# arkworks-rs/poly-commit

Measured on NVIDIA H100. Metric: MarlinKZG10/BLS12-381 commit+open polys/s at deg 2^20, higher is better.
Workload: dtype u32-limb Montgomery (Fq 381-bit x12, Fr 255-bit x8)

## Files before the change

poly-commit_b200/csrc/impl.cuh:

```cuda
#pragma once
#include <algorithm>
#include <initializer_list>
#include <memory>
#include <mutex>
#include <new>
#include <type_traits>
#include <vector>

#include "../../include/pcgpu.h"
#include "frops.cuh"
#include "host_ec.hpp"
#include "host_glv.hpp"
#include "ntt.cuh"
#include "ipa.cuh"
#include <chrono>
#include "msm.cuh"
#include "srs.cuh"
#include "wire.cuh"
#include "msm_small.cuh"
#include "peer.cuh"
#include "hash.cuh"
#include "sprs.cuh"
#include "field_ops.cuh"
#include "mlpc.cuh"
// ... 1984 lines not shown
#pragma unroll
      for (int j = 0; j < 8; j++) {
        uint32_t x = hi[(j + 3) & 7];
        lo[j] = mad_lo_cc(x, y, lo[j]);
        hi[j] = madc_hi(x, y, hi[j]);
      }
    }
    uint64_t acc = 0;
#pragma unroll
    for (int j = 0; j < 8; j++) acc ^= ((uint64_t)hi[j] << 32) | lo[j];
    sink[t] = acc;
  }
};

inline int measure_imad_peak_impl(pcgpu_ctx *ctx, double *ops_per_s) {
#ifdef PCGPU_EMUL
  (void)ctx; *ops_per_s = 0; return PCGPU_OK;
#else
  rt::stream_t st = ctx->stream;
  int rc;
  int dev = 0, sms = 0;
  if (cudaGetDevice(&dev) != cudaSuccess || cudaDeviceGetAttribute(&sms, cudaDevAttrMultiProcessorCount, dev) != cudaSuccess)
    return PCGPU_E_CUDA;
  const size_t threads = (size_t)sms * 2048;
  const uint32_t iters = 4096;
  uint64_t *sink;
  Staging io(ctx, 0);
  io.scratch(sink, threads * 8);
  if ((rc = io.upload())) return rc;
  cudaEvent_t e0, e1;
  cudaEventCreate(&e0); cudaEventCreate(&e1);
  if ((rc = rt::launch<256>(ImadPeakBody{sink, 64}, threads, st))) return rc;
  cudaEventRecord(e0, st);
  if ((rc = rt::launch<256>(ImadPeakBody{sink, iters}, threads, st))) return rc;
  cudaEventRecord(e1, st);
  if ((rc = rt::stream_sync(st))) return rc;
  float ms = 0; cudaEventElapsedTime(&ms, e0, e1);
  cudaEventDestroy(e0); cudaEventDestroy(e1);
  *ops_per_s = (double)threads * iters * 8.0 / (ms * 1e-3);
  return PCGPU_OK;
#endif
}

#define PCGPU_INST_PIPE(C, EXT)                                                                                            \
  EXT template int msm_device_planes<C>(pcgpu_ctx *, const MsmPlan &, const uint32_t *, const XYZZ<C> **, uint32_t **);  \
  EXT template int msm_to_host<C>(pcgpu_ctx *, const pcgpu_srs *, size_t, const uint32_t *, size_t, bool, host::HXYZZ<C> *); \
  EXT template int msm_issue<C>(pcgpu_ctx *, const pcgpu_srs *, size_t, const uint32_t *, size_t, bool, MsmPending<C> *);   \
  EXT template int msm_collect<C>(pcgpu_ctx *, MsmPending<C> *, host::HXYZZ<C> *);
#define PCGPU_INST_PAIR1(C, EXT)                                                                                           \
  EXT template int pcgpu::msm_pair_round_oneshot<C>(bool, const uint32_t *, const MsmGeom &, const uint32_t *, const Affine<C> *, uint32_t *, \
                                             const uint32_t *, uint32_t, uint32_t *, const uint32_t *, Affine<C> *, rt::stream_t);   \
  EXT template int pcgpu::msm_pair_oneshot_threads<C>(size_t *);
#define PCGPU_INST_ACC(C, EXT)                                                                                             \
  EXT template int pcgpu::msm_accumulate_launch<C>(const uint32_t *, const MsmGeom &, const uint32_t *, const uint32_t *, const uint32_t *, \
                                            const uint32_t *, XYZZ<C> *, uint32_t *, const Affine<C> *, rt::stream_t);
#define PCGPU_INST_REDUCE(C, EXT)                                                                                          \
  EXT template int pcgpu::msm_reduce_launch<C>(const MsmGeom &, const uint32_t *, const XYZZ<C> *, XYZZ<C> *, XYZZ<C> *, XYZZ<C> *,    \
                                        const uint32_t *, const uint32_t *, rt::stream_t);
#define PCGPU_INST_SMALL(C, EXT)                                                                                           \
  EXT template int msm_small_to_host<C>(pcgpu_ctx *, const MsmPlan &, const MsmSmallProblem<C> *, uint32_t, bool, host::HXYZZ<C> *);
#define PCGPU_INST_SRS(C, EXT)                                                                                             \
  EXT template int srs_register_impl<C>(pcgpu_ctx *, const void *, const uint8_t *, size_t, uint32_t, pcgpu_srs *);        \
  EXT template int msm_impl<C>(pcgpu_ctx *, const pcgpu_srs *, size_t, const void *, size_t, uint32_t, void *, uint8_t *, void *); \
  EXT template int g1_sum_impl<C>(pcgpu_ctx *, const void *, size_t, void *, uint8_t *);                                   \
  EXT template int fixed_base_impl<C>(pcgpu_ctx *, const void *, const void *, size_t, uint32_t, void *);                  \
  EXT template int kzg_commit_impl<C>(pcgpu_ctx *, const pcgpu_srs *, const void *, size_t, const pcgpu_srs *, const void *, \
                                      size_t, uint32_t, void *, uint8_t *);                                                \
  EXT template int kzg_open_impl<C>(pcgpu_ctx *, const pcgpu_srs *, const void *, size_t, const void *, const pcgpu_srs *, \
                                    const void *, size_t, uint32_t, void *, uint8_t *, void *); \
  EXT template int msm_batch_impl<C>(pcgpu_ctx *, const pcgpu_srs *, const void *, size_t, size_t, uint32_t, void *, uint8_t *); \
  EXT template int kzg_commit_open_impl<C>(pcgpu_ctx *, pcgpu_ctx *, const pcgpu_srs *, const void *, size_t, const void *, uint32_t, void *, uint8_t *, void *, uint8_t *); \
  EXT template int msm_peer_impl<C>(pcgpu_ctx *, const pcgpu_srs *, size_t, const void *, size_t, uint32_t, void *const *, uint32_t, uint32_t, uint64_t, void *, uint8_t *); \
  EXT template int hyrax_commit_impl<C>(pcgpu_ctx *, const pcgpu_srs *, uint32_t, const void *, const void *, uint32_t, void *, uint8_t *, pcgpu_hyrax *); \
  EXT template int hyrax_open_impl<C>(pcgpu_ctx *, const pcgpu_srs *, const pcgpu_hyrax *const *, size_t, uint32_t, const void *, const void *, \
                                      uint32_t, void *, uint8_t *, void *, void *); \
  EXT template int hyrax_check_impl<C>(pcgpu_ctx *, const pcgpu_srs *, uint32_t, size_t, const void *, const uint8_t *, const void *, const void *, \
                                       const uint8_t *, const void *, const void *, uint32_t, uint8_t *);
#define PCGPU_INST_FR(C, EXT)                                                                                              \
  EXT template int fr_from_mont_impl<C>(pcgpu_ctx *, const void *, void *, size_t, uint32_t);                              \
  EXT template int fr_axpy_impl<C>(pcgpu_ctx *, void *, const void *, const void *, size_t, uint32_t);                     \
  EXT template int fr_div_impl<C>(pcgpu_ctx *, const void *, size_t, const void *, void *, void *, uint32_t);              \
  EXT template int fr_ip_impl<C>(pcgpu_ctx *, const void *, const void *, size_t, void *, uint32_t);                       \
  EXT template int fr_row_mul_impl<C>(pcgpu_ctx *, const void *, const void *, size_t, size_t, void *, uint32_t);          \
  EXT template int fr_mul_impl<C>(pcgpu_ctx *, const void *, const void *, void *, size_t, uint32_t); \
  EXT template int selftest_field_impl<C>(pcgpu_ctx *, uint64_t, size_t, uint64_t *); \
  EXT template int diag_field_op_impl<C>(pcgpu_ctx *, int, int, const void *, const void *, void *, size_t); \
  EXT template int ntt_impl<C>(pcgpu_ctx *, const void *, size_t, uint32_t, uint32_t, void *); \
  EXT template int ntt_pass_impl<C>(pcgpu_ctx *, uint32_t, uint32_t, int, size_t, size_t, const void *, size_t, void *); \
  EXT template int ntt_batch_impl<C>(pcgpu_ctx *, const void *, size_t, size_t, uint32_t, uint32_t, void *); \
  EXT template int ntt_pass1_peer_impl<C>(pcgpu_ctx *, uint32_t, uint32_t, size_t, size_t, const void *, size_t, void *const *, uint32_t); \
  EXT template int lincode_hash_columns_impl<C>(pcgpu_ctx *, const void *, size_t, size_t, int, uint32_t, uint8_t *); \
  EXT template int lincode_commit_impl<C>(pcgpu_ctx *, const void *, size_t, size_t, uint32_t, int, uint32_t, void *, uint8_t *, uint8_t *, uint8_t *); \
  EXT template int brakedown_register_impl<C>(pcgpu_ctx *, uint64_t, uint64_t, uint64_t, const uint64_t *, const uint64_t *, \
                                              const uint64_t *const *, const uint64_t *const *, const void *const *, pcgpu_brakedown *); \
  EXT template int brakedown_commit_impl<C>(pcgpu_ctx *, const pcgpu_brakedown *, const void *, size_t, size_t, int, uint32_t, void *, \
                                            uint8_t *, uint8_t *, uint8_t *); \
  EXT template int fr_sprs_row_mul_impl<C>(pcgpu_ctx *, size_t, size_t, const uint64_t *, const uint64_t *, const void *, const void *, \
                                           size_t, uint32_t, void *);
#define PCGPU_INST_IPA(C, EXT)                                                                                             \
  EXT template int ipa_begin_impl<C>(pcgpu_ctx *, const void *, size_t, const void *, size_t, const void *, uint32_t, pcgpu_ipa *); \
  EXT template int ipa_round_lr_impl<C>(pcgpu_ctx *, pcgpu_ctx *, pcgpu_ipa *, const void *, void *, uint8_t *, void *, uint8_t *); \
  EXT template int ipa_round_fold_impl<C>(pcgpu_ctx *, pcgpu_ipa *, const void *, const void *); \
  EXT template int ipa_finish_impl<C>(pcgpu_ctx *, pcgpu_ipa *, void *, void *); \
  EXT template int ipa_check_final_key_impl<C>(pcgpu_ctx *, const pcgpu_srs *, const void *, uint32_t, void *, uint8_t *); \
  EXT template int g1_serialize_impl<C>(pcgpu_ctx *, const void *, const uint8_t *, size_t, uint32_t, uint8_t *); \
  EXT template int g1_deserialize_impl<C>(pcgpu_ctx *, const uint8_t *, size_t, uint32_t, void *, uint8_t *, size_t *, int *); \
  EXT template int g1_sample_generators_impl<C>(pcgpu_ctx *, const uint8_t *, size_t, uint64_t, size_t, uint32_t, void *);
#define PCGPU_INST_G2(C, EXT)                                                                                              \
  EXT template int srs_register_impl<C>(pcgpu_ctx *, const void *, const uint8_t *, size_t, uint32_t, pcgpu_srs *);        \
  EXT template int msm_impl<C>(pcgpu_ctx *, const pcgpu_srs *, size_t, const void *, size_t, uint32_t, void *, uint8_t *, void *); \
  EXT template int fixed_base_impl<C>(pcgpu_ctx *, const void *, const void *, size_t, uint32_t, void *);                  \
// ... 16 lines not shown
```

poly-commit_b200/csrc/msm.cuh:

```cuda
#pragma once
#include "ec.cuh"
#include "rt.cuh"

namespace pcgpu {

struct alignas(16) u32x4 { uint32_t x, y, z, w; };

struct MsmGeom {
  uint32_t n;
  uint32_t c;
  uint32_t W;
  uint32_t S;
  uint32_t G;
  uint32_t NB;
  uint32_t TB;
  uint32_t L;
  uint32_t seg_len;
  uint32_t nseg;
  uint32_t scalar_bits;
  uint32_t scalars_mont;
  uint64_t table_stride;
  uint64_t base_off;
  uint32_t affine_rounds;
  uint32_t h_split;
// ... 135 lines not shown
    size_t lo = t * SCAN_CHUNK, hi = lo + SCAN_CHUNK < n ? lo + SCAN_CHUNK : n;
    uint32_t run = partial[t];
    for (size_t i = lo; i < hi; i++) { uint32_t v = in[i]; out[i] = run; run += v; }
    if (t + 1 == m) out[n] = partial[m];
  }
};

enum { SCAN_BLOCK = 1024, SCAN_PER = 8, SCAN_BLOCK_MAX = 1 << 17 };
struct ScanBlockBody {
  const uint32_t *in; size_t n; uint32_t *out;
  PCGPU_KERNEL_DEV void operator()(size_t, uint32_t *smem) const {
    uint32_t *a = smem, *b = smem + SCAN_BLOCK, *carry = smem + 2 * SCAN_BLOCK;
    PCGPU_BLOCK_FOR(t, 1) { carry[0] = 0; }
    PCGPU_BLOCK_SYNC();
    const size_t tile = (size_t)SCAN_BLOCK * SCAN_PER;
    for (size_t base = 0; base < n; base += tile) {
      PCGPU_BLOCK_FOR(t, SCAN_BLOCK) {
        const size_t lo = base + (size_t)t * SCAN_PER;
        uint32_t sum = 0;
        for (uint32_t k = 0; k < SCAN_PER; k++) if (lo + k < n) sum += in[lo + k];
        a[t] = sum;
      }
      PCGPU_BLOCK_SYNC();
      uint32_t *x = a, *y = b;
      for (uint32_t d = 1; d < SCAN_BLOCK; d <<= 1) {
        PCGPU_BLOCK_FOR(t, SCAN_BLOCK) { y[t] = x[t] + (t >= d ? x[t - d] : 0u); }
        PCGPU_BLOCK_SYNC();
        uint32_t *tmp = x; x = y; y = tmp;
      }
      PCGPU_BLOCK_FOR(t, SCAN_BLOCK) {
        const size_t lo = base + (size_t)t * SCAN_PER;
        uint32_t run = carry[0] + (t ? x[t - 1] : 0u);
        for (uint32_t k = 0; k < SCAN_PER; k++) if (lo + k < n) { uint32_t v = in[lo + k]; out[lo + k] = run; run += v; }
      }
      PCGPU_BLOCK_SYNC();
      PCGPU_BLOCK_FOR(t, 1) { carry[0] += x[SCAN_BLOCK - 1]; }
      PCGPU_BLOCK_SYNC();
    }
    PCGPU_BLOCK_FOR(t, 1) { out[n] = carry[0]; }
  }
};

inline size_t scan_scratch_words(size_t n) { return (n + SCAN_CHUNK - 1) / SCAN_CHUNK + 2; }
inline int exclusive_scan_u32(const uint32_t *in, size_t n, uint32_t *out, uint32_t *scratch, rt::stream_t st) {
  size_t m = (n + SCAN_CHUNK - 1) / SCAN_CHUNK;
  if (m == 0) { return rt::dev_memset(out, 0, sizeof(uint32_t), st); }
  if (n <= SCAN_BLOCK_MAX) return rt::launch_blocks<SCAN_BLOCK>(ScanBlockBody{in, n, out}, 1, (2 * SCAN_BLOCK + 4) * sizeof(uint32_t), st);
  int rc;
  if ((rc = rt::launch<128>(ScanChunkSumBody{in, n, scratch}, m, st))) return rc;
  if ((rc = rt::launch<32>(ScanPartialsBody{scratch, m}, 1, st))) return rc;
  return rt::launch<128>(ScanApplyBody{in, n, scratch, out, m}, m, st);
}

struct TaskCountBody {
  const uint32_t *offsets; uint32_t L; uint32_t *ntasks; uint32_t heavy_min; uint32_t *heavy_count; uint32_t *heavy_list;
  PCGPU_KERNEL_DEV void operator()(size_t b) const {
    uint32_t cnt = offsets[b + 1] - offsets[b];
    uint32_t nt = (cnt + L - 1) / L;
    ntasks[b] = nt;
    if (nt > heavy_min) heavy_list[rt::atomic_add(heavy_count, 1u)] = (uint32_t)b;
  }
};
struct TaskFillBody {
  const uint32_t *task_off; uint32_t *task_bucket;
  PCGPU_KERNEL_DEV void operator()(size_t b) const {
    uint32_t lo = task_off[b], hi = task_off[b + 1];
    for (uint32_t t = lo; t < hi; t++) task_bucket[t] = (uint32_t)b;
  }
};

template <class C>
PCGPU_DEV Affine<C> load_affine(const Affine<C> *p) {
  constexpr int N = coord_words<typename C::F>();
  const u32x4 *q = reinterpret_cast<const u32x4 *>(p);
  Affine<C> a;
  uint32_t tmp[2 * N];
#pragma unroll
  for (int j = 0; j < 2 * N / 4; j++) { u32x4 v = q[j]; tmp[4 * j] = v.x; tmp[4 * j + 1] = v.y; tmp[4 * j + 2] = v.z; tmp[4 * j + 3] = v.w; }
#pragma unroll
  for (int j = 0; j < N; j++) {
    if constexpr (C::EXT == 1) { a.x.l[j] = tmp[j]; a.y.l[j] = tmp[N + j]; }
    else { coord_word(a.x, j) = tmp[j]; coord_word(a.y, j) = tmp[N + j]; }
  }
  return a;
}

template <class C>
PCGPU_DEV const uint32_t *table_record(const uint32_t *tables, size_t idx, const MsmGeom &g) { return tables + idx * g.pt_words; }
template <class C>
PCGPU_DEV Affine<C> load_table_point(const uint32_t *tables, size_t idx, const MsmGeom &g) {
  constexpr int N = coord_words<typename C::F>();
  const uint32_t *rec = tables + idx * g.pt_words;
  const u32x4 *qx = reinterpret_cast<const u32x4 *>(rec), *qy = reinterpret_cast<const u32x4 *>(rec + g.y_words);
  Affine<C> a;
#pragma unroll
  for (int j = 0; j < N / 4; j++) {
    u32x4 v = qx[j]; coord_word(a.x, 4 * j) = v.x; coord_word(a.x, 4 * j + 1) = v.y; coord_word(a.x, 4 * j + 2) = v.z; coord_word(a.x, 4 * j + 3) = v.w;
    u32x4 w = qy[j]; coord_word(a.y, 4 * j) = w.x; coord_word(a.y, 4 * j + 1) = w.y; coord_word(a.y, 4 * j + 2) = w.z; coord_word(a.y, 4 * j + 3) = w.w;
  }
  return a;
}
template <class C>
PCGPU_DEV void store_table_point(uint32_t *tables, size_t idx, uint32_t pt_words, uint32_t y_words, const Affine<C> &a) {
  constexpr int N = coord_words<typename C::F>();
  uint32_t *rec = tables + idx * pt_words;
  u32x4 *qx = reinterpret_cast<u32x4 *>(rec), *qy = reinterpret_cast<u32x4 *>(rec + y_words);
#pragma unroll
  for (int j = 0; j < N / 4; j++) {
    u32x4 v; v.x = coord_word(a.x, 4 * j); v.y = coord_word(a.x, 4 * j + 1); v.z = coord_word(a.x, 4 * j + 2); v.w = coord_word(a.x, 4 * j + 3); qx[j] = v;
    u32x4 w; w.x = coord_word(a.y, 4 * j); w.y = coord_word(a.y, 4 * j + 1); w.z = coord_word(a.y, 4 * j + 2); w.w = coord_word(a.y, 4 * j + 3); qy[j] = w;
  }
}
template <class C> constexpr uint32_t aligned_pt_words() { return C::Fq::N == 12 ? 32u : 2u * C::Fq::N; }
template <class C> constexpr uint32_t aligned_y_words() { return C::Fq::N == 12 ? 16u : (uint32_t)C::Fq::N; }

template <class C>
PCGPU_DEV void store_xyzz(XYZZ<C> *dst, const XYZZ<C> &p) {
  constexpr int N = coord_words<typename C::F>();
  u32x4 *q = reinterpret_cast<u32x4 *>(dst);
  const uint32_t *src = reinterpret_cast<const uint32_t *>(&p);
#pragma unroll
  for (int j = 0; j < 4 * N / 4; j++) { u32x4 v; v.x = src[4 * j]; v.y = src[4 * j + 1]; v.z = src[4 * j + 2]; v.w = src[4 * j + 3]; q[j] = v; }
}

template <class C>
PCGPU_DEV XYZZ<C> load_xyzz(const XYZZ<C> *src) {
  constexpr int N = coord_words<typename C::F>();
  const u32x4 *q = reinterpret_cast<const u32x4 *>(src);
  XYZZ<C> p;
  uint32_t *dst = reinterpret_cast<uint32_t *>(&p);
#pragma unroll
  for (int j = 0; j < 4 * N / 4; j++) { u32x4 v = q[j]; dst[4 * j] = v.x; dst[4 * j + 1] = v.y; dst[4 * j + 2] = v.z; dst[4 * j + 3] = v.w; }
  return p;
}

template <class C>
struct MsmAccumulateBody {
  const uint32_t *tables; MsmGeom g;
  const uint32_t *offsets;
  const uint32_t *task_off;
  const uint32_t *task_bucket;
  const uint32_t *entries;
  XYZZ<C> *partial;
  uint32_t *queue;
  const Affine<C> *pts;
  PCGPU_KERNEL_DEV void operator()(size_t) const {
    const uint32_t total = task_off[g.TB];
    for (;;) {
      uint32_t t = rt::next_task(queue);
      if (t - (t & 31u) >= total) break;
      if (t >= total) continue;
      uint32_t b = task_bucket[t];
      uint32_t t0 = task_off[b], T = task_off[b + 1] - t0, j = t - t0;
      uint32_t base = offsets[b], cnt = offsets[b + 1] - base;
      uint32_t lo = base + (uint32_t)(((uint64_t)cnt * j) / T);
      uint32_t hi = base + (uint32_t)(((uint64_t)cnt * (j + 1)) / T);
      XYZZ<C> acc = XYZZ<C>::inf();
      if (pts) {
        for (uint32_t e = lo; e < hi; e++) { Affine<C> a = load_affine<C>(pts + e); xyzz_madd<C>(acc, a, false); }
      } else {
        for (uint32_t e = lo; e < hi; e++) {
          uint32_t v = entries[e];
          uint32_t grp = (v & ~ENTRY_SIGN) >> ENTRY_GROUP_SHIFT;
          size_t idx = (size_t)grp * g.table_stride + g.base_off + (v & ENTRY_IDX_MASK);
          Affine<C> a = load_table_point<C>(tables, idx, g);
          xyzz_madd<C>(acc, a, (v & ENTRY_SIGN) != 0);
        }
      }
      store_xyzz<C>(partial + t, acc);
    }
  }
};

enum { HEAVY_BUCKET_TASKS = 8, HEAVY_BLOCK = 128, HEAVY_GRID = 64, REDUCE_BLOCK = 128 };

template <class C>
#ifdef __CUDACC__
__device__ __noinline__
#else
inline
#endif
void xyzz_add_ool(XYZZ<C> &acc, const XYZZ<C> &p) { xyzz_add<C>(acc, p); }

template <class C>
struct MsmHeavyBucketBody {
  const uint32_t *task_off; const XYZZ<C> *partial; XYZZ<C> *buckets; const uint32_t *heavy_count; const uint32_t *heavy_list;
  PCGPU_KERNEL_DEV void operator()(size_t blk, uint32_t *smem) const {
    XYZZ<C> *sh = reinterpret_cast<XYZZ<C> *>(smem);
    const uint32_t nheavy = *heavy_count;
    for (uint32_t hb = (uint32_t)blk; hb < nheavy; hb += HEAVY_GRID) {
      const uint32_t b = heavy_list[hb], t0 = task_off[b], t1 = task_off[b + 1];
      PCGPU_BLOCK_FOR(i, HEAVY_BLOCK) {
        XYZZ<C> acc = XYZZ<C>::inf();
#pragma unroll 1
        for (uint32_t q = t0 + i; q < t1; q += HEAVY_BLOCK) { XYZZ<C> p = load_xyzz<C>(partial + q); xyzz_add_ool<C>(acc, p); }
        sh[i] = acc;
      }
      PCGPU_BLOCK_SYNC();
#pragma unroll 1
      for (uint32_t half = HEAVY_BLOCK / 2; half >= 1; half >>= 1) {
        PCGPU_BLOCK_FOR(i, half) { XYZZ<C> x = sh[i], y = sh[i + half]; xyzz_add_ool<C>(x, y); sh[i] = x; }
        PCGPU_BLOCK_SYNC();
      }
      PCGPU_BLOCK_FOR(i, 1) { store_xyzz<C>(buckets + b, sh[0]); }
      PCGPU_BLOCK_SYNC();
    }
  }
};

template <class C>
PCGPU_KERNEL_DEV void block_tree_sum(XYZZ<C> *sh) {
#pragma unroll 1
  for (uint32_t half = REDUCE_BLOCK / 2; half >= 1; half >>= 1) {
    PCGPU_BLOCK_FOR(i, half) { XYZZ<C> x = sh[i], y = sh[i + half]; xyzz_add_ool<C>(x, y); sh[i] = x; }
    PCGPU_BLOCK_SYNC();
  }
}

template <class C>
struct MsmRowReduceBody {
  const uint32_t *task_off; const XYZZ<C> *partial; XYZZ<C> *buckets; XYZZ<C> *Rv;
  uint32_t NB, rows, cols;
  PCGPU_KERNEL_DEV void operator()(size_t blk, uint32_t *smem) const {
    XYZZ<C> *sh = reinterpret_cast<XYZZ<C> *>(smem);
    const uint32_t s = (uint32_t)(blk / rows), hi = (uint32_t)(blk % rows);
    PCGPU_BLOCK_FOR(t, REDUCE_BLOCK) {
      XYZZ<C> acc = XYZZ<C>::inf();
#pragma unroll 1
      for (uint32_t lo = t; lo < cols; lo += REDUCE_BLOCK) {
        const size_t b = (size_t)s * NB + (size_t)hi * cols + lo;
        const uint32_t t0 = task_off[b], t1 = task_off[b + 1];
        XYZZ<C> bs;
        if (t1 - t0 > HEAVY_BUCKET_TASKS) bs = load_xyzz<C>(buckets + b);
        else {
          bs = XYZZ<C>::inf();
#pragma unroll 1
          for (uint32_t q = t0; q < t1; q++) { XYZZ<C> p = load_xyzz<C>(partial + q); xyzz_add_ool<C>(bs, p); }
          store_xyzz<C>(buckets + b, bs);
        }
        xyzz_add_ool<C>(acc, bs);
      }
      sh[t] = acc;
    }
    PCGPU_BLOCK_SYNC();
    block_tree_sum<C>(sh);
    PCGPU_BLOCK_FOR(i, 1) { store_xyzz<C>(Rv + blk, sh[0]); }
  }
};
template <class C>
struct MsmColReduceBody {
  const XYZZ<C> *buckets; XYZZ<C> *Cv;
  uint32_t NB, rows, cols;
  PCGPU_KERNEL_DEV void operator()(size_t blk, uint32_t *smem) const {
    XYZZ<C> *sh = reinterpret_cast<XYZZ<C> *>(smem);
    const uint32_t s = (uint32_t)(blk / cols), lo = (uint32_t)(blk % cols);
    PCGPU_BLOCK_FOR(t, REDUCE_BLOCK) {
      XYZZ<C> acc = XYZZ<C>::inf();
#pragma unroll 1
      for (uint32_t hi = t; hi < rows; hi += REDUCE_BLOCK) {
        XYZZ<C> p = load_xyzz<C>(buckets + (size_t)s * NB + (size_t)hi * cols + lo);
        xyzz_add_ool<C>(acc, p);
      }
      sh[t] = acc;
    }
    PCGPU_BLOCK_SYNC();
    block_tree_sum<C>(sh);
    PCGPU_BLOCK_FOR(i, 1) { store_xyzz<C>(Cv + blk, sh[0]); }
  }
};
template <class C>
struct MsmPlaneReduceBody {
  const XYZZ<C> *Rv, *Cv; XYZZ<C> *plane_out;
  uint32_t rows, cols, bits_c, bits_r;
  PCGPU_KERNEL_DEV void operator()(size_t blk, uint32_t *smem) const {
    XYZZ<C> *sh = reinterpret_cast<XYZZ<C> *>(smem);
    const uint32_t per = bits_c + bits_r;
    const uint32_t s = (uint32_t)(blk / per), j = (uint32_t)(blk % per);
    const bool col = j < bits_c;
    const XYZZ<C> *vals = col ? Cv + (size_t)s * cols : Rv + (size_t)s * rows;
    const uint32_t cnt = col ? cols : rows, wofs = col ? 1u : 0u, bit = col ? j : j - bits_c;
    PCGPU_BLOCK_FOR(t, REDUCE_BLOCK) {
      XYZZ<C> acc = XYZZ<C>::inf();
#pragma unroll 1
      for (uint32_t k = t; k < cnt; k += REDUCE_BLOCK)
        if (((k + wofs) >> bit) & 1) { XYZZ<C> p = load_xyzz<C>(vals + k); xyzz_add_ool<C>(acc, p); }
      sh[t] = acc;
    }
// ... 22 lines not shown
  MsmGeom g{};
  g.n = (uint32_t)n; g.c = c;
  g.W = (scalar_bits + c - 1) / c;
  g.G = groups < 1 ? 1 : groups;
  g.S = (g.W + g.G - 1) / g.G;
  g.NB = 1u << (c - 1);
  g.TB = g.S * g.NB;
  g.L = L;
  g.seg_len = 16;
  g.nseg = (g.NB + g.seg_len - 1) / g.seg_len;
  g.scalar_bits = scalar_bits; g.scalars_mont = mont ? 1 : 0;
  g.table_stride = table_stride; g.base_off = base_off;
  g.h_split = (c - 1) / 2;
  return g;
}

struct MsmPlan {
  uint32_t path;
  uint64_t n;
  uint32_t split;
  MsmGeom g;
  const uint32_t *tables;
  size_t wave;
  uint32_t T;
};

inline size_t msm_plane_scratch_elems(const MsmGeom &g) {
  size_t cols = (size_t)1 << g.h_split, rows = g.NB >> g.h_split;
  return (size_t)g.S * (rows + cols);
}

enum {
  MSM_ERR_RANGE = 0,
  MSM_ERR_QUEUE = 8,
  MSM_ERR_HEAVY = 12,
  MSM_ERR_WORDS = 16,
};

#ifndef PCGPU_PAIR_MIN_BLOCKS
#define PCGPU_PAIR_MIN_BLOCKS 4
#endif
enum { PAIR_MIN_BLOCKS = PCGPU_PAIR_MIN_BLOCKS };

template <class C>
int msm_pair_round_oneshot(bool round0, const uint32_t *tables, const MsmGeom &g, const uint32_t *entries, const Affine<C> *in,
                           uint32_t *src, const uint32_t *off_out, uint32_t T, uint32_t *prefix, const uint32_t *pow2, Affine<C> *out,
                           rt::stream_t st) {
  if (round0) return rt::launch_occ<128, PAIR_MIN_BLOCKS>(MsmAffinePairBody<C, true>{tables, g, entries, nullptr, src, off_out, T, prefix, pow2, out}, T, st);
  return rt::launch_occ<128, PAIR_MIN_BLOCKS>(MsmAffinePairBody<C, false>{tables, g, entries, in, src, off_out, T, prefix, pow2, out}, T, st);
}
template <class C> int msm_pair_oneshot_threads(size_t *out) { return rt::resident_threads_occ<128, PAIR_MIN_BLOCKS, MsmAffinePairBody<C, true>>(out); }

template <class C>
int msm_accumulate_launch(const uint32_t *tables, const MsmGeom &g, const uint32_t *offsets, const uint32_t *task_off,
                          const uint32_t *task_bucket, const uint32_t *entries, XYZZ<C> *partial, uint32_t *queue, const Affine<C> *pts,
                          rt::stream_t st) {
  return rt::launch_persistent<128>(MsmAccumulateBody<C>{tables, g, offsets, task_off, task_bucket, entries, partial, queue, pts}, st);
}

template <class C>
int msm_reduce_launch(const MsmGeom &g, const uint32_t *task_off, const XYZZ<C> *partial, XYZZ<C> *buckets, XYZZ<C> *planes,
                      XYZZ<C> *plane_out, const uint32_t *heavy_count, const uint32_t *heavy_list, rt::stream_t st) {
  const uint32_t h = g.h_split, cols = 1u << h, rows = g.NB >> h, bits_c = h + 1, bits_r = g.c - 1 - h;
  const size_t smem = REDUCE_BLOCK * sizeof(XYZZ<C>);
  XYZZ<C> *Rv = planes, *Cv = planes + (size_t)g.S * rows;
  int rc;
  if ((rc = rt::launch_blocks<HEAVY_BLOCK>(MsmHeavyBucketBody<C>{task_off, partial, buckets, heavy_count, heavy_list}, HEAVY_GRID,
                                           HEAVY_BLOCK * sizeof(XYZZ<C>), st))) return rc;
  if ((rc = rt::launch_blocks<REDUCE_BLOCK>(MsmRowReduceBody<C>{task_off, partial, buckets, Rv, g.NB, rows, cols}, (size_t)g.S * rows, smem, st))) return rc;
  if ((rc = rt::launch_blocks<REDUCE_BLOCK>(MsmColReduceBody<C>{buckets, Cv, g.NB, rows, cols}, (size_t)g.S * cols, smem, st))) return rc;
  return rt::launch_blocks<REDUCE_BLOCK>(MsmPlaneReduceBody<C>{Rv, Cv, plane_out, rows, cols, bits_c, bits_r}, (size_t)g.S * (bits_c + bits_r), smem, st);
}

template <class C, class Prof>
inline int msm_run(const MsmPlan &plan, const uint32_t *d_scalars, rt::Arena &arena, const XYZZ<C> **d_planes,
                   uint32_t **d_err_out, rt::stream_t st, Prof &prof, const uint32_t *pow2) {
  using QF = Fp<typename C::Fq>;
  const MsmGeom &g = plan.g;
  const size_t max_entries = (size_t)g.n * g.W, max_tasks = max_entries / g.L + g.TB + 1;
  const size_t bound0 = max_entries / 2 + g.TB + 1, bound1 = bound0 / 2 + g.TB + 1;
  const bool pair_rounds = C::EXT == 1 && g.affine_rounds;
  uint32_t *counts, *offsets, *cursor, *ntasks, *task_off, *task_bucket, *entries, *scratch, *err;
  XYZZ<C> *partial, *buckets, *planes, *plane_out;
  uint32_t *offA = nullptr, *offB = nullptr, *cnt = nullptr, *src = nullptr;
  QF *prefix = nullptr; Affine<C> *ptsA = nullptr, *ptsB = nullptr;
  int rc = arena.carve([&](auto &&buf) {
    buf(counts, g.TB + 2); buf(offsets, g.TB + 2); buf(cursor, g.TB + 2); buf(ntasks, g.TB + 2); buf(task_off, g.TB + 2);
    buf(task_bucket, max_tasks); buf(entries, max_entries + 1); buf(scratch, scan_scratch_words(g.TB + 1)); buf(err, MSM_ERR_WORDS);
    buf(partial, max_tasks); buf(buckets, g.TB); buf(planes, msm_plane_scratch_elems(g));
    buf(plane_out, (size_t)g.S * 2 * g.c);
    if (pair_rounds) {
      buf(offA, g.TB + 2); buf(offB, g.TB + 2); buf(cnt, g.TB + 2); buf(src, bound0);
      buf(prefix, bound0 + (1u << 20));
      buf(ptsA, bound0); buf(ptsB, bound1);
    }
  });
  if (rc) return rc;
  *d_err_out = err; *d_planes = plane_out;

  prof.begin(0, st);
  if ((rc = rt::dev_memset(counts, 0, (g.TB + 2) * sizeof(uint32_t), st))) return rc;
  if ((rc = rt::dev_memset(err, 0, MSM_ERR_WORDS * sizeof(uint32_t), st))) return rc;
  if ((rc = rt::launch<256>(MsmCountBody<C>{d_scalars, g, counts, err + MSM_ERR_RANGE}, g.n, st))) return rc;
  prof.end(0, st);

  prof.begin(1, st);
  if ((rc = exclusive_scan_u32(counts, g.TB, offsets, scratch, st))) return rc;
  if ((rc = rt::copy_d2d(cursor, offsets, (g.TB + 1) * sizeof(uint32_t), st))) return rc;
  prof.end(1, st);

  prof.begin(2, st);
  if ((rc = rt::launch<256>(MsmScatterBody<C>{d_scalars, g, cursor, entries}, g.n, st))) return rc;
  prof.end(2, st);

  const Affine<C> *pts = nullptr;
  if constexpr (C::EXT == 1) if (pair_rounds) {
    prof.begin(11, st);
    const uint32_t *off_in = offsets;
    size_t bound = max_entries;
    for (uint32_t r = 0; r < g.affine_rounds; r++) {
      uint32_t *off_out = (r & 1) ? offB : offA;
      Affine<C> *out = (r & 1) ? ptsB : ptsA;
      const Affine<C> *in = (r & 1) ? ptsA : ptsB;
      bound = bound / 2 + g.TB + 1;
      if ((rc = rt::launch<256>(PairCountBody{off_in, cnt}, g.TB, st))) return rc;
      if ((rc = exclusive_scan_u32(cnt, g.TB, off_out, scratch, st))) return rc;
      if ((rc = rt::launch<256>(PairPlanBody{off_in, off_out, g.TB, src}, bound, st))) return rc;
      if (r == 0) prof.begin(12, st);
      rc = msm_pair_round_oneshot<C>(r == 0, plan.tables, g, entries, in, src, off_out, plan.T, (uint32_t *)prefix, pow2, out, st);
      if (rc) return rc;
      if (r == 0) prof.end(12, st);
      off_in = off_out;
      pts = out;
    }
    prof.end(11, st);
    offsets = const_cast<uint32_t *>(off_in);
  }

  prof.begin(3, st);
  if ((rc = rt::dev_memset(err + MSM_ERR_HEAVY, 0, 4, st))) return rc;
  if ((rc = rt::launch<256>(TaskCountBody{offsets, g.L, ntasks, HEAVY_BUCKET_TASKS, err + MSM_ERR_HEAVY, cursor}, g.TB, st))) return rc;
  if ((rc = exclusive_scan_u32(ntasks, g.TB, task_off, scratch, st))) return rc;
  if ((rc = rt::launch<256>(TaskFillBody{task_off, task_bucket}, g.TB, st))) return rc;
  prof.end(3, st);

  prof.begin(4, st);
  if ((rc = msm_accumulate_launch<C>(plan.tables, g, offsets, task_off, task_bucket, entries, partial, err + MSM_ERR_QUEUE, pts, st))) return rc;
  prof.end(4, st);

  prof.begin(5, st);
  if ((rc = msm_reduce_launch<C>(g, task_off, partial, buckets, planes, plane_out, err + MSM_ERR_HEAVY, cursor, st))) return rc;
  prof.end(5, st);
  return rt::OK;
}

}
```

poly-commit_b200/csrc/rt.cuh:

```cuda
#pragma once
#include <stddef.h>
#include <stdint.h>
#include <stdlib.h>
#include <string.h>
#include <atomic>
#include <type_traits>

#ifndef PCGPU_EMUL
#include <cuda_runtime.h>
#endif

namespace pcgpu {
namespace rt {

enum : int {
  OK = 0,
  E_CUDA = -1,
  E_OOM = -2,
  E_BADARG = -3,
  E_LEN = -4,
  E_RANGE = -5,
  E_DEGREE = -6,
  E_HIDING = -7,
};

inline std::atomic<uint64_t> &launch_counter() { static std::atomic<uint64_t> c{0}; return c; }

#ifdef PCGPU_EMUL
typedef void *stream_t;
inline int dev_malloc(void **p, size_t bytes) { *p = ::malloc(bytes ? bytes : 1); return *p ? OK : E_OOM; }
inline void dev_free(void *p) { ::free(p); }
inline int dev_memset(void *p, int v, size_t bytes, stream_t) { memset(p, v, bytes); return OK; }
inline int copy_h2d(void *d, const void *h, size_t bytes, stream_t) { memcpy(d, h, bytes); return OK; }
inline int copy_d2h(void *h, const void *d, size_t bytes, stream_t) { memcpy(h, d, bytes); return OK; }
inline int copy_d2d(void *d, const void *s, size_t bytes, stream_t) { memmove(d, s, bytes); return OK; }
inline int stream_sync(stream_t) { return OK; }
inline int last_error() { return OK; }
typedef int event_t;
inline int event_create(event_t *e) { *e = 0; return OK; }
inline void event_destroy(event_t) {}
inline int event_record(event_t, stream_t) { return OK; }
inline int stream_wait_event(stream_t, event_t) { return OK; }
inline int host_alloc_pinned(void **p, size_t bytes) { *p = ::malloc(bytes ? bytes : 1); return *p ? OK : E_OOM; }
inline void host_free_pinned(void *p) { ::free(p); }

template <int BLOCK, class Body>
inline int launch(const Body &body, size_t n, stream_t) {
  for (size_t i = 0; i < n; i++) body(i);
  return OK;
}
template <class T> inline T atomic_add(T *p, T v) { T o = *p; *p = o + v; return o; }
template <class T> inline T atomic_or(T *p, T v) { T o = *p; *p = o | v; return o; }
#define PCGPU_KERNEL_DEV inline
inline uint32_t next_task(uint32_t *counter) { return atomic_add(counter, 1u); }
template <int BLOCK, class Body>
inline int launch_persistent(const Body &body, stream_t) { body(0); return OK; }
template <int BLOCK, int MINB, class Body> inline int launch_occ(const Body &body, size_t n, stream_t s) { return launch<BLOCK>(body, n, s); }
template <int BLOCK, int MINB, class Body> inline int resident_threads_occ(size_t *out) { *out = 48; return OK; }
#define PCGPU_BLOCK_FOR(i, n) for (uint32_t i = 0; i < (uint32_t)(n); i++)
#define PCGPU_BLOCK_SYNC() do { } while (0)
#define PCGPU_WARP_ANY(x) (x)
template <int BLOCK, class Body>
inline int launch_blocks(const Body &body, size_t nblocks, size_t smem_bytes, stream_t) {
  uint32_t *smem = (uint32_t *)::malloc(smem_bytes ? smem_bytes : 16);
  if (!smem) return E_OOM;
  for (size_t b = 0; b < nblocks; b++) body(b, smem);
  ::free(smem);
  return OK;
}

template <int BLOCK, int MINB, class Body>
inline int launch_blocks_occ(const Body &body, size_t nblocks, size_t smem_bytes, stream_t s) { return launch_blocks<BLOCK>(body, nblocks, smem_bytes, s); }

#else
typedef cudaStream_t stream_t;

inline int map_cuda(cudaError_t e) {
  if (e == cudaSuccess) return OK;
  if (e == cudaErrorMemoryAllocation) return E_OOM;
  return E_CUDA;
}
inline int dev_malloc(void **p, size_t bytes) { return map_cuda(cudaMalloc(p, bytes ? bytes : 1)); }
inline void dev_free(void *p) { if (p) cudaFree(p); }
inline int dev_memset(void *p, int v, size_t bytes, stream_t s) { return map_cuda(cudaMemsetAsync(p, v, bytes, s)); }
inline int copy_h2d(void *d, const void *h, size_t bytes, stream_t s) { return map_cuda(cudaMemcpyAsync(d, h, bytes, cudaMemcpyHostToDevice, s)); }
inline int copy_d2h(void *h, const void *d, size_t bytes, stream_t s) { return map_cuda(cudaMemcpyAsync(h, d, bytes, cudaMemcpyDeviceToHost, s)); }
inline int copy_d2d(void *d, const void *s_, size_t bytes, stream_t s) { return map_cuda(cudaMemcpyAsync(d, s_, bytes, cudaMemcpyDeviceToDevice, s)); }
inline int stream_sync(stream_t s) { return map_cuda(cudaStreamSynchronize(s)); }
inline int last_error() { return map_cuda(cudaGetLastError()); }
typedef cudaEvent_t event_t;
inline int event_create(event_t *e) { return map_cuda(cudaEventCreateWithFlags(e, cudaEventDisableTiming)); }
inline void event_destroy(event_t e) { cudaEventDestroy(e); }
inline int event_record(event_t e, stream_t s) { return map_cuda(cudaEventRecord(e, s)); }
inline int stream_wait_event(stream_t s, event_t e) { return map_cuda(cudaStreamWaitEvent(s, e, 0)); }
inline int host_alloc_pinned(void **p, size_t bytes) { return map_cuda(cudaMallocHost(p, bytes ? bytes : 1)); }
inline void host_free_pinned(void *p) { if (p) cudaFreeHost(p); }

template <class Body, int BLOCK>
__global__ void __launch_bounds__(BLOCK) run_kernel(const Body body, size_t n) {
  size_t tid = (size_t)blockIdx.x * BLOCK + threadIdx.x;
  if (tid < n) body(tid);
}

template <int BLOCK, class Body>
inline int launch(const Body &body, size_t n, stream_t s) {
  if (n == 0) return OK;
  size_t grid = (n + BLOCK - 1) / BLOCK;
  run_kernel<Body, BLOCK><<<(unsigned)grid, BLOCK, 0, s>>>(body, n);
  launch_counter().fetch_add(1, std::memory_order_relaxed);
// ... 22 lines not shown
    if (e == cudaSuccess) e = cudaOccupancyMaxActiveBlocksPerMultiprocessor(&per_sm, run_kernel_occ<Body, BLOCK, MINB>, BLOCK, 0);
    if (e != cudaSuccess) return map_cuda(e);
    cached = (size_t)sms * (per_sm > 0 ? per_sm : 1) * BLOCK;
  }
  *out = cached;
  return OK;
}
#define PCGPU_BLOCK_FOR(i, n) for (uint32_t i = threadIdx.x; i < (uint32_t)(n); i += blockDim.x)
#define PCGPU_BLOCK_SYNC() __syncthreads()
#define PCGPU_WARP_ANY(x) __any_sync(0xffffffffu, (x))
template <class Body, int BLOCK>
__global__ void __launch_bounds__(BLOCK) run_block_kernel(const Body body) {
  extern __shared__ uint4 pcgpu_smem[];
  body((size_t)blockIdx.x, reinterpret_cast<uint32_t *>(pcgpu_smem));
}
template <int BLOCK, class Body>
inline int launch_blocks(const Body &body, size_t nblocks, size_t smem_bytes, stream_t s) {
  if (nblocks == 0) return OK;
  if (smem_bytes > 48 * 1024) {
    cudaError_t e = cudaFuncSetAttribute(run_block_kernel<Body, BLOCK>, cudaFuncAttributeMaxDynamicSharedMemorySize, (int)smem_bytes);
    if (e != cudaSuccess) return map_cuda(e);
  }
  run_block_kernel<Body, BLOCK><<<(unsigned)nblocks, BLOCK, smem_bytes, s>>>(body);
  launch_counter().fetch_add(1, std::memory_order_relaxed);
  return last_error();
}
template <class Body, int BLOCK, int MINB>
__global__ void __launch_bounds__(BLOCK, MINB) run_block_kernel_occ(const Body body) {
  extern __shared__ uint4 pcgpu_smem[];
  body((size_t)blockIdx.x, reinterpret_cast<uint32_t *>(pcgpu_smem));
}
template <int BLOCK, int MINB, class Body>
inline int launch_blocks_occ(const Body &body, size_t nblocks, size_t smem_bytes, stream_t s) {
  if (nblocks == 0) return OK;
  if (smem_bytes > 48 * 1024) {
    cudaError_t e = cudaFuncSetAttribute(run_block_kernel_occ<Body, BLOCK, MINB>, cudaFuncAttributeMaxDynamicSharedMemorySize, (int)smem_bytes);
    if (e != cudaSuccess) return map_cuda(e);
  }
  run_block_kernel_occ<Body, BLOCK, MINB><<<(unsigned)nblocks, BLOCK, smem_bytes, s>>>(body);
  launch_counter().fetch_add(1, std::memory_order_relaxed);
  return last_error();
}
__device__ __forceinline__ uint32_t next_task(uint32_t *counter) {
  uint32_t lane = threadIdx.x & 31, base = 0;
  if (lane == 0) base = atomicAdd(counter, 32u);
  base = __shfl_sync(0xffffffffu, base, 0);
  return base + lane;
}
template <class Body, int BLOCK>
__global__ void __launch_bounds__(BLOCK) run_persistent_kernel(const Body body) {
  body((size_t)blockIdx.x * BLOCK + threadIdx.x);
}
template <int BLOCK, class Body>
inline int launch_persistent(const Body &body, stream_t s) {
  static int grid = 0;
  if (grid == 0) {
    int dev = 0, sms = 0, per_sm = 0;
    cudaError_t e = cudaGetDevice(&dev);
    if (e == cudaSuccess) e = cudaDeviceGetAttribute(&sms, cudaDevAttrMultiProcessorCount, dev);
    if (e == cudaSuccess) e = cudaOccupancyMaxActiveBlocksPerMultiprocessor(&per_sm, run_persistent_kernel<Body, BLOCK>, BLOCK, 0);
    if (e != cudaSuccess) return map_cuda(e);
    grid = sms * (per_sm > 0 ? per_sm : 1);
  }
  run_persistent_kernel<Body, BLOCK><<<grid, BLOCK, 0, s>>>(body);
  launch_counter().fetch_add(1, std::memory_order_relaxed);
  return last_error();
}
template <class T> __device__ __forceinline__ T atomic_add(T *p, T v) { return atomicAdd(p, v); }
template <class T> __device__ __forceinline__ T atomic_or(T *p, T v) { return atomicOr(p, v); }
#define PCGPU_KERNEL_DEV __device__ __forceinline__
#endif

struct Arena {
  char *base = nullptr;
  size_t cap = 0;
  int reserve(size_t bytes) {
    if (bytes <= cap) return OK;
    if (base) dev_free(base);
    base = nullptr; cap = 0;
    int rc = dev_malloc((void **)&base, bytes);
    if (rc) return rc;
    cap = bytes;
    return OK;
  }
  template <class List> int carve(const List &list) {
    size_t used = 0;
    list([&](auto *&p, size_t count) { used += padded(sizeof *p, count); });
    int rc = reserve(used);
    if (rc) return rc;
    used = 0;
    list([&](auto *&p, size_t count) {
      p = reinterpret_cast<std::remove_reference_t<decltype(p)>>(base + used);
      used += padded(sizeof *p, count);
    });
    return OK;
  }
  static size_t padded(size_t elem, size_t count) { size_t b = elem * count; return ((b ? b : 1) + 255) & ~(size_t)255; }
  void release() { if (base) dev_free(base); base = nullptr; cap = 0; }
};

}
}
```

Before: 74.52.

## Split MSM bucket accumulation into equal flat chunks across persistent lanes

```diff
diff --git a/poly-commit_b200/csrc/impl.cuh b/poly-commit_b200/csrc/impl.cuh
--- a/poly-commit_b200/csrc/impl.cuh
+++ b/poly-commit_b200/csrc/impl.cuh
@@ -2060,11 +2060,12 @@
                                              const uint32_t *, uint32_t, uint32_t *, const uint32_t *, Affine<C> *, rt::stream_t);   \
   EXT template int pcgpu::msm_pair_oneshot_threads<C>(size_t *);
 #define PCGPU_INST_ACC(C, EXT)                                                                                             \
-  EXT template int pcgpu::msm_accumulate_launch<C>(const uint32_t *, const MsmGeom &, const uint32_t *, const uint32_t *, const uint32_t *, \
-                                            const uint32_t *, XYZZ<C> *, uint32_t *, const Affine<C> *, rt::stream_t);
+  EXT template int pcgpu::msm_accumulate_launch<C>(const uint32_t *, const MsmGeom &, const uint32_t *, const uint32_t *, XYZZ<C> *, \
+                                            uint32_t *, const Affine<C> *, uint32_t, rt::stream_t);                        \
+  EXT template int pcgpu::msm_tail_chunks<C>(uint32_t *);
 #define PCGPU_INST_REDUCE(C, EXT)                                                                                          \
-  EXT template int pcgpu::msm_reduce_launch<C>(const MsmGeom &, const uint32_t *, const XYZZ<C> *, XYZZ<C> *, XYZZ<C> *, XYZZ<C> *,    \
-                                        const uint32_t *, const uint32_t *, rt::stream_t);
+  EXT template int pcgpu::msm_reduce_launch<C>(const MsmGeom &, const uint32_t *, uint32_t, const XYZZ<C> *, XYZZ<C> *, XYZZ<C> *, \
+                                        XYZZ<C> *, const uint32_t *, const uint32_t *, rt::stream_t);
 #define PCGPU_INST_SMALL(C, EXT)                                                                                           \
   EXT template int msm_small_to_host<C>(pcgpu_ctx *, const MsmPlan &, const MsmSmallProblem<C> *, uint32_t, bool, host::HXYZZ<C> *);
 #define PCGPU_INST_SRS(C, EXT)                                                                                             \
diff --git a/poly-commit_b200/csrc/msm.cuh b/poly-commit_b200/csrc/msm.cuh
--- a/poly-commit_b200/csrc/msm.cuh
+++ b/poly-commit_b200/csrc/msm.cuh
@@ -211,20 +211,23 @@
   return rt::launch<128>(ScanApplyBody{in, n, scratch, out, m}, m, st);
 }
 
-struct TaskCountBody {
-  const uint32_t *offsets; uint32_t L; uint32_t *ntasks; uint32_t heavy_min; uint32_t *heavy_count; uint32_t *heavy_list;
+enum { TAIL_CHUNKS_PER_LANE = 1, HEAVY_BUCKET_TASKS = 8 };
+
+PCGPU_DEV uint32_t tail_chunk_len(uint32_t M, uint32_t chunks, uint32_t L) {
+  const uint32_t s = M / chunks + (M % chunks != 0), lo = L / 2;
+  return s > lo ? s : lo;
+}
+PCGPU_DEV void tail_partials(const uint32_t *offsets, uint32_t b, uint32_t s, uint32_t *t0, uint32_t *t1) {
+  const uint32_t lo = offsets[b], hi = offsets[b + 1];
+  *t0 = lo / s + b;
+  *t1 = lo < hi ? (hi - 1) / s + b + 1 : *t0;
+}
+PCGPU_DEV bool tail_heavy(uint32_t cnt, uint32_t L) { return (cnt + L - 1) / L > HEAVY_BUCKET_TASKS; }
+
+struct HeavyListBody {
+  const uint32_t *offsets; uint32_t L; uint32_t *heavy_count; uint32_t *heavy_list;
   PCGPU_KERNEL_DEV void operator()(size_t b) const {
-    uint32_t cnt = offsets[b + 1] - offsets[b];
-    uint32_t nt = (cnt + L - 1) / L;
-    ntasks[b] = nt;
-    if (nt > heavy_min) heavy_list[rt::atomic_add(heavy_count, 1u)] = (uint32_t)b;
-  }
-};
-struct TaskFillBody {
-  const uint32_t *task_off; uint32_t *task_bucket;
-  PCGPU_KERNEL_DEV void operator()(size_t b) const {
-    uint32_t lo = task_off[b], hi = task_off[b + 1];
-    for (uint32_t t = lo; t < hi; t++) task_bucket[t] = (uint32_t)b;
+    if (tail_heavy(offsets[b + 1] - offsets[b], L)) heavy_list[rt::atomic_add(heavy_count, 1u)] = (uint32_t)b;
   }
 };
 
@@ -297,41 +300,45 @@
 struct MsmAccumulateBody {
   const uint32_t *tables; MsmGeom g;
   const uint32_t *offsets;
-  const uint32_t *task_off;
-  const uint32_t *task_bucket;
   const uint32_t *entries;
   XYZZ<C> *partial;
   uint32_t *queue;
   const Affine<C> *pts;
+  uint32_t chunks;
   PCGPU_KERNEL_DEV void operator()(size_t) const {
-    const uint32_t total = task_off[g.TB];
+    const uint32_t M = offsets[g.TB], s = tail_chunk_len(M, chunks, g.L), total = M / s + (M % s != 0);
     for (;;) {
-      uint32_t t = rt::next_task(queue);
+      const uint32_t t = rt::next_task(queue);
       if (t - (t & 31u) >= total) break;
       if (t >= total) continue;
-      uint32_t b = task_bucket[t];
-      uint32_t t0 = task_off[b], T = task_off[b + 1] - t0, j = t - t0;
-      uint32_t base = offsets[b], cnt = offsets[b + 1] - base;
-      uint32_t lo = base + (uint32_t)(((uint64_t)cnt * j) / T);
-      uint32_t hi = base + (uint32_t)(((uint64_t)cnt * (j + 1)) / T);
+      const uint32_t lo = t * s, hi = M - lo > s ? lo + s : M;
+      uint32_t b = 0, bh = g.TB;
+      while (bh - b > 1) { const uint32_t mid = (b + bh) >> 1; if (offsets[mid] <= lo) b = mid; else bh = mid; }
+      uint32_t next = offsets[b + 1];
       XYZZ<C> acc = XYZZ<C>::inf();
-      if (pts) {
-        for (uint32_t e = lo; e < hi; e++) { Affine<C> a = load_affine<C>(pts + e); xyzz_madd<C>(acc, a, false); }
-      } else {
-        for (uint32_t e = lo; e < hi; e++) {
-          uint32_t v = entries[e];
-          uint32_t grp = (v & ~ENTRY_SIGN) >> ENTRY_GROUP_SHIFT;
-          size_t idx = (size_t)grp * g.table_stride + g.base_off + (v & ENTRY_IDX_MASK);
-          Affine<C> a = load_table_point<C>(tables, idx, g);
-          xyzz_madd<C>(acc, a, (v & ENTRY_SIGN) != 0);
+      for (uint32_t e = lo; e < hi; e++) {
+        if (e == next) {
+          store_xyzz<C>(partial + t + b, acc);
+          acc = XYZZ<C>::inf();
+          do next = offsets[++b + 1]; while (next == e);
         }
-      }
-      store_xyzz<C>(partial + t, acc);
-    }
-  }
-};
-
-enum { HEAVY_BUCKET_TASKS = 8, HEAVY_BLOCK = 128, HEAVY_GRID = 64, REDUCE_BLOCK = 128 };
+        Affine<C> a;
+        bool neg = false;
+        if (pts) a = load_affine<C>(pts + e);
+        else {
+          const uint32_t v = entries[e];
+          const uint32_t grp = (v & ~ENTRY_SIGN) >> ENTRY_GROUP_SHIFT;
+          a = load_table_point<C>(tables, (size_t)grp * g.table_stride + g.base_off + (v & ENTRY_IDX_MASK), g);
+          neg = (v & ENTRY_SIGN) != 0;
+        }
+        xyzz_madd<C>(acc, a, neg);
+      }
+      store_xyzz<C>(partial + t + b, acc);
+    }
+  }
+};
+
+enum { HEAVY_BLOCK = 128, HEAVY_GRID = 64, REDUCE_BLOCK = 128 };
 
 template <class C>
 #ifdef __CUDACC__
@@ -343,12 +350,15 @@
 
 template <class C>
 struct MsmHeavyBucketBody {
-  const uint32_t *task_off; const XYZZ<C> *partial; XYZZ<C> *buckets; const uint32_t *heavy_count; const uint32_t *heavy_list;
+  const uint32_t *offsets; uint32_t TB, L, chunks; const XYZZ<C> *partial; XYZZ<C> *buckets; const uint32_t *heavy_count;
+  const uint32_t *heavy_list;
   PCGPU_KERNEL_DEV void operator()(size_t blk, uint32_t *smem) const {
     XYZZ<C> *sh = reinterpret_cast<XYZZ<C> *>(smem);
-    const uint32_t nheavy = *heavy_count;
+    const uint32_t nheavy = *heavy_count, s = tail_chunk_len(offsets[TB], chunks, L);
     for (uint32_t hb = (uint32_t)blk; hb < nheavy; hb += HEAVY_GRID) {
-      const uint32_t b = heavy_list[hb], t0 = task_off[b], t1 = task_off[b + 1];
+      uint32_t t0, t1;
+      const uint32_t b = heavy_list[hb];
+      tail_partials(offsets, b, s, &t0, &t1);
       PCGPU_BLOCK_FOR(i, HEAVY_BLOCK) {
         XYZZ<C> acc = XYZZ<C>::inf();
 #pragma unroll 1
@@ -378,20 +388,21 @@
 
 template <class C>
 struct MsmRowReduceBody {
-  const uint32_t *task_off; const XYZZ<C> *partial; XYZZ<C> *buckets; XYZZ<C> *Rv;
+  const uint32_t *offsets; uint32_t TB, L, chunks; const XYZZ<C> *partial; XYZZ<C> *buckets; XYZZ<C> *Rv;
   uint32_t NB, rows, cols;
   PCGPU_KERNEL_DEV void operator()(size_t blk, uint32_t *smem) const {
     XYZZ<C> *sh = reinterpret_cast<XYZZ<C> *>(smem);
-    const uint32_t s = (uint32_t)(blk / rows), hi = (uint32_t)(blk % rows);
+    const uint32_t s = (uint32_t)(blk / rows), hi = (uint32_t)(blk % rows), len = tail_chunk_len(offsets[TB], chunks, L);
     PCGPU_BLOCK_FOR(t, REDUCE_BLOCK) {
       XYZZ<C> acc = XYZZ<C>::inf();
 #pragma unroll 1
       for (uint32_t lo = t; lo < cols; lo += REDUCE_BLOCK) {
-        const size_t b = (size_t)s * NB + (size_t)hi * cols + lo;
-        const uint32_t t0 = task_off[b], t1 = task_off[b + 1];
+        const uint32_t b = s * NB + hi * cols + lo;
         XYZZ<C> bs;
-        if (t1 - t0 > HEAVY_BUCKET_TASKS) bs = load_xyzz<C>(buckets + b);
+        if (tail_heavy(offsets[b + 1] - offsets[b], L)) bs = load_xyzz<C>(buckets + b);
         else {
+          uint32_t t0, t1;
+          tail_partials(offsets, b, len, &t0, &t1);
           bs = XYZZ<C>::inf();
 #pragma unroll 1
           for (uint32_t q = t0; q < t1; q++) { XYZZ<C> p = load_xyzz<C>(partial + q); xyzz_add_ool<C>(bs, p); }
@@ -520,22 +531,29 @@
 template <class C> int msm_pair_oneshot_threads(size_t *out) { return rt::resident_threads_occ<128, PAIR_MIN_BLOCKS, MsmAffinePairBody<C, true>>(out); }
 
 template <class C>
-int msm_accumulate_launch(const uint32_t *tables, const MsmGeom &g, const uint32_t *offsets, const uint32_t *task_off,
-                          const uint32_t *task_bucket, const uint32_t *entries, XYZZ<C> *partial, uint32_t *queue, const Affine<C> *pts,
-                          rt::stream_t st) {
-  return rt::launch_persistent<128>(MsmAccumulateBody<C>{tables, g, offsets, task_off, task_bucket, entries, partial, queue, pts}, st);
-}
-
-template <class C>
-int msm_reduce_launch(const MsmGeom &g, const uint32_t *task_off, const XYZZ<C> *partial, XYZZ<C> *buckets, XYZZ<C> *planes,
-                      XYZZ<C> *plane_out, const uint32_t *heavy_count, const uint32_t *heavy_list, rt::stream_t st) {
+int msm_tail_chunks(uint32_t *out) {
+  size_t lanes = 0;
+  int rc = rt::persistent_threads<128, MsmAccumulateBody<C>>(&lanes);
+  *out = (uint32_t)(TAIL_CHUNKS_PER_LANE * lanes);
+  return rc;
+}
+
+template <class C>
+int msm_accumulate_launch(const uint32_t *tables, const MsmGeom &g, const uint32_t *offsets, const uint32_t *entries, XYZZ<C> *partial,
+                          uint32_t *queue, const Affine<C> *pts, uint32_t chunks, rt::stream_t st) {
+  return rt::launch_persistent<128>(MsmAccumulateBody<C>{tables, g, offsets, entries, partial, queue, pts, chunks}, st);
+}
+
+template <class C>
+int msm_reduce_launch(const MsmGeom &g, const uint32_t *offsets, uint32_t chunks, const XYZZ<C> *partial, XYZZ<C> *buckets,
+                      XYZZ<C> *planes, XYZZ<C> *plane_out, const uint32_t *heavy_count, const uint32_t *heavy_list, rt::stream_t st) {
   const uint32_t h = g.h_split, cols = 1u << h, rows = g.NB >> h, bits_c = h + 1, bits_r = g.c - 1 - h;
   const size_t smem = REDUCE_BLOCK * sizeof(XYZZ<C>);
   XYZZ<C> *Rv = planes, *Cv = planes + (size_t)g.S * rows;
   int rc;
-  if ((rc = rt::launch_blocks<HEAVY_BLOCK>(MsmHeavyBucketBody<C>{task_off, partial, buckets, heavy_count, heavy_list}, HEAVY_GRID,
+  if ((rc = rt::launch_blocks<HEAVY_BLOCK>(MsmHeavyBucketBody<C>{offsets, g.TB, g.L, chunks, partial, buckets, heavy_count, heavy_list}, HEAVY_GRID,
                                            HEAVY_BLOCK * sizeof(XYZZ<C>), st))) return rc;
-  if ((rc = rt::launch_blocks<REDUCE_BLOCK>(MsmRowReduceBody<C>{task_off, partial, buckets, Rv, g.NB, rows, cols}, (size_t)g.S * rows, smem, st))) return rc;
+  if ((rc = rt::launch_blocks<REDUCE_BLOCK>(MsmRowReduceBody<C>{offsets, g.TB, g.L, chunks, partial, buckets, Rv, g.NB, rows, cols}, (size_t)g.S * rows, smem, st))) return rc;
   if ((rc = rt::launch_blocks<REDUCE_BLOCK>(MsmColReduceBody<C>{buckets, Cv, g.NB, rows, cols}, (size_t)g.S * cols, smem, st))) return rc;
   return rt::launch_blocks<REDUCE_BLOCK>(MsmPlaneReduceBody<C>{Rv, Cv, plane_out, rows, cols, bits_c, bits_r}, (size_t)g.S * (bits_c + bits_r), smem, st);
 }
@@ -545,17 +563,20 @@
                    uint32_t **d_err_out, rt::stream_t st, Prof &prof, const uint32_t *pow2) {
   using QF = Fp<typename C::Fq>;
   const MsmGeom &g = plan.g;
-  const size_t max_entries = (size_t)g.n * g.W, max_tasks = max_entries / g.L + g.TB + 1;
+  const size_t max_entries = (size_t)g.n * g.W;
   const size_t bound0 = max_entries / 2 + g.TB + 1, bound1 = bound0 / 2 + g.TB + 1;
   const bool pair_rounds = C::EXT == 1 && g.affine_rounds;
-  uint32_t *counts, *offsets, *cursor, *ntasks, *task_off, *task_bucket, *entries, *scratch, *err;
+  uint32_t *counts, *offsets, *cursor, *entries, *scratch, *err;
   XYZZ<C> *partial, *buckets, *planes, *plane_out;
   uint32_t *offA = nullptr, *offB = nullptr, *cnt = nullptr, *src = nullptr;
   QF *prefix = nullptr; Affine<C> *ptsA = nullptr, *ptsB = nullptr;
-  int rc = arena.carve([&](auto &&buf) {
-    buf(counts, g.TB + 2); buf(offsets, g.TB + 2); buf(cursor, g.TB + 2); buf(ntasks, g.TB + 2); buf(task_off, g.TB + 2);
-    buf(task_bucket, max_tasks); buf(entries, max_entries + 1); buf(scratch, scan_scratch_words(g.TB + 1)); buf(err, MSM_ERR_WORDS);
-    buf(partial, max_tasks); buf(buckets, g.TB); buf(planes, msm_plane_scratch_elems(g));
+  uint32_t chunks = 0;
+  int rc = msm_tail_chunks<C>(&chunks);
+  if (rc) return rc;
+  rc = arena.carve([&](auto &&buf) {
+    buf(counts, g.TB + 2); buf(offsets, g.TB + 2); buf(cursor, g.TB + 2);
+    buf(entries, max_entries + 1); buf(scratch, scan_scratch_words(g.TB + 1)); buf(err, MSM_ERR_WORDS);
+    buf(partial, (size_t)chunks + g.TB + 1); buf(buckets, g.TB); buf(planes, msm_plane_scratch_elems(g));
     buf(plane_out, (size_t)g.S * 2 * g.c);
     if (pair_rounds) {
       buf(offA, g.TB + 2); buf(offB, g.TB + 2); buf(cnt, g.TB + 2); buf(src, bound0);
@@ -607,17 +628,15 @@
 
   prof.begin(3, st);
   if ((rc = rt::dev_memset(err + MSM_ERR_HEAVY, 0, 4, st))) return rc;
-  if ((rc = rt::launch<256>(TaskCountBody{offsets, g.L, ntasks, HEAVY_BUCKET_TASKS, err + MSM_ERR_HEAVY, cursor}, g.TB, st))) return rc;
-  if ((rc = exclusive_scan_u32(ntasks, g.TB, task_off, scratch, st))) return rc;
-  if ((rc = rt::launch<256>(TaskFillBody{task_off, task_bucket}, g.TB, st))) return rc;
+  if ((rc = rt::launch<256>(HeavyListBody{offsets, g.L, err + MSM_ERR_HEAVY, cursor}, g.TB, st))) return rc;
   prof.end(3, st);
 
   prof.begin(4, st);
-  if ((rc = msm_accumulate_launch<C>(plan.tables, g, offsets, task_off, task_bucket, entries, partial, err + MSM_ERR_QUEUE, pts, st))) return rc;
+  if ((rc = msm_accumulate_launch<C>(plan.tables, g, offsets, entries, partial, err + MSM_ERR_QUEUE, pts, chunks, st))) return rc;
   prof.end(4, st);
 
   prof.begin(5, st);
-  if ((rc = msm_reduce_launch<C>(g, task_off, partial, buckets, planes, plane_out, err + MSM_ERR_HEAVY, cursor, st))) return rc;
+  if ((rc = msm_reduce_launch<C>(g, offsets, chunks, partial, buckets, planes, plane_out, err + MSM_ERR_HEAVY, cursor, st))) return rc;
   prof.end(5, st);
   return rt::OK;
 }
diff --git a/poly-commit_b200/csrc/rt.cuh b/poly-commit_b200/csrc/rt.cuh
--- a/poly-commit_b200/csrc/rt.cuh
+++ b/poly-commit_b200/csrc/rt.cuh
@@ -55,6 +55,7 @@
 inline uint32_t next_task(uint32_t *counter) { return atomic_add(counter, 1u); }
 template <int BLOCK, class Body>
 inline int launch_persistent(const Body &body, stream_t) { body(0); return OK; }
+template <int BLOCK, class Body> inline int persistent_threads(size_t *out) { *out = 48; return OK; }
 template <int BLOCK, int MINB, class Body> inline int launch_occ(const Body &body, size_t n, stream_t s) { return launch<BLOCK>(body, n, s); }
 template <int BLOCK, int MINB, class Body> inline int resident_threads_occ(size_t *out) { *out = 48; return OK; }
 #define PCGPU_BLOCK_FOR(i, n) for (uint32_t i = 0; i < (uint32_t)(n); i++)
@@ -183,7 +184,7 @@
   body((size_t)blockIdx.x * BLOCK + threadIdx.x);
 }
 template <int BLOCK, class Body>
-inline int launch_persistent(const Body &body, stream_t s) {
+inline int persistent_grid(int *out) {
   static int grid = 0;
   if (grid == 0) {
     int dev = 0, sms = 0, per_sm = 0;
@@ -193,6 +194,19 @@
     if (e != cudaSuccess) return map_cuda(e);
     grid = sms * (per_sm > 0 ? per_sm : 1);
   }
+  *out = grid;
+  return OK;
+}
+template <int BLOCK, class Body>
+inline int persistent_threads(size_t *out) {
+  int grid = 0, rc = persistent_grid<BLOCK, Body>(&grid);
+  *out = (size_t)grid * BLOCK;
+  return rc;
+}
+template <int BLOCK, class Body>
+inline int launch_persistent(const Body &body, stream_t s) {
+  int grid = 0;
+  if (int rc = persistent_grid<BLOCK, Body>(&grid)) return rc;
   run_persistent_kernel<Body, BLOCK><<<grid, BLOCK, 0, s>>>(body);
   launch_counter().fetch_add(1, std::memory_order_relaxed);
   return last_error();
```

New measurement: 75.45, median of 6. 1.01x the previous value.
